# codelibs/ranklib

Measured on AMD Instinct MI355X. Metric: boosting rounds/sec (LambdaMART -ranker 6, NDCG@10), higher is better.
Workload: dtype int64 fixed-point histograms + f64 lambdas/scores (f32 leaf chains as in the Java)

## Files before the change

ranklib_amd/csrc/rl_internal.h:

```cpp
#pragma once
#include <hip/hip_runtime.h>
#include <stdint.h>

#include <string>
#include <vector>

#include "../../include/rlhip.h"

namespace rl {

constexpr int kThreads = 256;
constexpr int kWave = 64;
constexpr int kFinThreads = 320;
constexpr int kLog2Chunk = 14;
constexpr int kChunk = 1 << kLog2Chunk;
#ifndef RL_NODE_CHUNK
#define RL_NODE_CHUNK 8192
#endif
constexpr int kNodeChunk = RL_NODE_CHUNK;
constexpr int kMinChunk = 512;
#ifndef RL_HIST_DOCS
#define RL_HIST_DOCS 2
#endif
constexpr int kHistDocs = RL_HIST_DOCS;
#ifndef RL_LOOKBACK2
#define RL_LOOKBACK2 1
#endif
#ifndef RL_HIST_PREFETCH
#define RL_HIST_PREFETCH 0
#endif
constexpr int kHistFG = 16;
#ifndef RL_PART_TILE
#define RL_PART_TILE 2048
#endif
constexpr int kPartTile = RL_PART_TILE;
constexpr int kMaxBins = 4096;
constexpr int kHistLdsStride = 264;
constexpr int kHistLdsBytes = 64 * 1024;
#ifndef RL_KSPEC
#define RL_KSPEC 4
#endif
constexpr int kSpec = RL_KSPEC;
constexpr int kLambdaWaveCap = 384;
constexpr int kLambdaBlockCap = 5000;
#ifndef RL_RANK_SHORT
#define RL_RANK_SHORT 384
#endif
constexpr int kRankShort = RL_RANK_SHORT;
constexpr int kLambdaFusedMaxK = 16;

struct NodeRec {
    int32_t start, count;
    int32_t buf, parent;
    int32_t left, right;
    int32_t best_f, best_t;
    double  best_S;
    double  deviance;
    double  sum_response;
    double  sq_response;
    long long tot_hi; unsigned long long tot_lo;
    long long sq;
    float   output; int32_t gcount;
    int32_t pl, pr;
    int32_t fid;
    int32_t prepared;
    int32_t best_cl, tie;
    unsigned long long ph;
    long long best_hi; unsigned long long best_lo;
};

struct SlotRec {
// ... 166 lines not shown
```

ranklib_amd/csrc/rl_k_rank.inc:

```

namespace rl {

template <int G>
__device__ __forceinline__ void group_sync()
{
    if (G > kWave) __syncthreads();
    else { __builtin_amdgcn_fence(__ATOMIC_ACQ_REL, "workgroup"); __builtin_amdgcn_wave_barrier(); }
}

constexpr int kRankLdsPerDoc = 20;
struct RankArgs {
    const double *scores; const float *labels; const int *qoff; const double *ideal; const double *disc;
    double *ss; float *sl; int *srel; int *sidx;
    double *ndcg; int k;
    int metric;
    int *aux_i; double *aux_a, *aux_b;
    double err_max;
    const int *rd_ext;
};

__device__ __forceinline__ double err_R(int rel, double mx) { return (double)java_pow2m1(rel) / mx; }

__device__ __forceinline__ bool metric_binary_view(int metric) { return metric == RL_METRIC_MAP || metric == RL_METRIC_P || metric == RL_METRIC_RR; }
__device__ void rank_metric(const RankArgs &a, int qi, int cur, int n, int size, const int *s_rel)
{
    const bool is_map = a.metric == RL_METRIC_MAP;
    {
        double res = 0.0;
        if (a.metric == RL_METRIC_NDCG) {
            const double ideal = a.ideal[qi];
            if (n > 0 && ideal > 0.0) {
                double dcg = 0;
                for (int i = 0; i < size; i++) dcg += gain_of(s_rel[i]) * a.disc[i];
// ... 18 lines not shown
            int first = -1, second = -1;
            for (int i = 0; i < rsize && second < 0; i++)
                if (s_rel[i]) { if (first < 0) first = i; else second = i; }
            res = (first < 0) ? 0.0 : (double)(1.0f / (float)(first + 1));
            if (a.aux_i) { a.aux_i[2 * qi] = first; a.aux_i[2 * qi + 1] = second; }
        } else {
            double sc = 0.0, p = 1.0;
            for (int i = 1; i <= size; i++) { const double R = err_R(s_rel[i - 1], a.err_max); sc += p * R / i; p *= (1.0 - R); }
            res = sc;
            if (a.aux_a) {
                const int ssize = (n > a.k) ? a.k : n;
                double pp = 1.0;
                for (int i = 0; i < ssize; i++) {
                    const double R = err_R(s_rel[i], a.err_max), np = pp * (1.0 - R);
                    pp *= np;
                    a.aux_a[cur + i] = R; a.aux_b[cur + i] = np;
                }
            }
        }
        a.ndcg[qi] = res;
    }
}

template <int G, int CAP>
__device__ void rank_query(const RankArgs &a, int qi, int tid, double *s_raw, int *s_rel, float *s_lab, int *s_idx)
{
    int cur = a.qoff[qi], n = a.qoff[qi + 1] - cur;
    if (G >= kWave) {
        cur = __builtin_amdgcn_readfirstlane(cur); n = __builtin_amdgcn_readfirstlane(n);
    }
    for (int i = tid; i < n; i += G) s_raw[i] = a.scores[cur + i];
    group_sync<G>();
    int size = a.k;
    if (a.k > n || a.k <= 0) size = n;
    const bool is_map = a.metric == RL_METRIC_MAP, bin_view = metric_binary_view(a.metric);
    constexpr int PER = (CAP + G - 1) / G;
    double v[PER]; float l[PER]; int pos[PER];
#pragma unroll
    for (int u = 0; u < PER; u++) {
        const int r = tid + u * G;
        pos[u] = 0; v[u] = 0.0; l[u] = 0.f;
        if (G >= kWave) {
            const int rb = __builtin_amdgcn_readfirstlane(r);
            if (rb >= n) break;
            v[u] = (r < n) ? s_raw[r] : 0.0;
            const int j0 = rb, j1 = min(rb + 64, n);
            int p = 0;
#pragma unroll 8
            for (int j = 0; j < j0; j++) p += (s_raw[j] >= v[u]) ? 1 : 0;
#pragma unroll 8
            for (int j = j0; j < j1; j++) { const double x = s_raw[j]; p += ((x > v[u]) || (x == v[u] && j < r)) ? 1 : 0; }
#pragma unroll 8
            for (int j = j1; j < n; j++) p += (s_raw[j] > v[u]) ? 1 : 0;
            pos[u] = p;
            if (r < n) l[u] = a.labels[cur + r];
        } else if (r < n) {
            v[u] = s_raw[r];
            int p = 0;
            for (int j = 0; j < n; j++) { const double x = s_raw[j]; p += (x > v[u]) || (x == v[u] && j < r); }
            pos[u] = p; l[u] = a.labels[cur + r];
        }
    }
    group_sync<G>();
#pragma unroll
    for (int u = 0; u < PER; u++) {
        const int r = tid + u * G;
        if (r < n) {
            s_raw[pos[u]] = v[u]; s_rel[pos[u]] = bin_view ? (l[u] > 0.f ? 1 : 0) : (int)l[u];
            if (a.ss) { s_lab[pos[u]] = l[u]; s_idx[pos[u]] = r; }
        }
    }
    group_sync<G>();
    if (a.ss)
        for (int i = tid; i < n; i += G) { const float lv = s_lab[i]; a.ss[cur + i] = s_raw[i]; a.sl[cur + i] = lv; a.srel[cur + i] = (int)lv; a.sidx[cur + i] = s_idx[i]; }
    group_sync<G>();
    if (is_map) {
        if (tid == 0) { int count = 0; for (int i = 0; i < n; i++) { const int r = s_rel[i]; count += r; s_rel[i] = (count << 1) | r; } }
        group_sync<G>();
        for (int i = tid; i < n; i += G) {
            const int e = s_rel[i], cnt = e >> 1;
            if (a.aux_i) a.aux_i[cur + i] = cnt;
            s_raw[i] = (e & 1) ? ((double)cnt) / (i + 1) : 0.0;
        }
        group_sync<G>();
        if (tid == 0) {
            double ap = 0.0;
            for (int i = 0; i < n; i++) ap += s_raw[i];
            const int count = (n > 0) ? (s_rel[n - 1] >> 1) : 0;
            const int rdc = a.rd_ext ? a.rd_ext[qi] : count;
            a.ndcg[qi] = (rdc == 0) ? 0.0 : ap / rdc;
        }
        return;
    }
    if (G >= kWave && size <= kWave && (a.metric == RL_METRIC_NDCG || a.metric == RL_METRIC_DCG)) {
        if (tid < kWave) {
            const double term = (tid < size) ? gain_of(s_rel[tid]) * a.disc[tid] : 0.0;
            const double ideal = (a.metric == RL_METRIC_NDCG) ? a.ideal[qi] : 1.0;
            double dcg = 0;
            for (int i = 0; i < size; i++) dcg += readlane_f64(term, i);
            double res = dcg;
            if (a.metric == RL_METRIC_NDCG) res = (n > 0 && ideal > 0.0) ? dcg / ideal : 0.0;
            if (tid == 0) a.ndcg[qi] = res;
        }
        return;
    }
    if (tid == 0) rank_metric(a, qi, cur, n, size, s_rel);
}

__global__ __launch_bounds__(kThreads) void k_rank_wave(const RankArgs a, const int *qlist, int nq, int cap)
{
    constexpr int CAP = kLambdaWaveCap;
    extern __shared__ unsigned char smem_raw[];
    const int wave = threadIdx.x >> 6;
    const int slot = blockIdx.x * 4 + wave;
    if (slot >= nq) return;
    const int qi = qlist ? qlist[slot] : slot;
    unsigned char *base = smem_raw + (size_t)wave * ((size_t)cap * kRankLdsPerDoc);
    rank_query<kWave, CAP>(a, qi, lane_id(), (double *)base, (int *)(base + (size_t)cap * 8), (float *)(base + (size_t)cap * 12), (int *)(base + (size_t)cap * 16));
}

constexpr int kRankTinyDocs = 16, kRankTinyGroups = 16;
__global__ __launch_bounds__(kRankTinyDocs * kRankTinyGroups) void k_rank_tiny(const RankArgs a, const int *qlist, int nq)
{
    __shared__ unsigned char sm[kRankTinyGroups * kRankTinyDocs * kRankLdsPerDoc];
    const int grp = threadIdx.x / kRankTinyDocs;
    const int slot = blockIdx.x * kRankTinyGroups + grp;
    if (slot >= nq) return;
    unsigned char *base = sm + (size_t)grp * (kRankTinyDocs * kRankLdsPerDoc);
    rank_query<kRankTinyDocs, kRankTinyDocs>(a, qlist[slot], threadIdx.x % kRankTinyDocs, (double *)base, (int *)(base + kRankTinyDocs * 8), (float *)(base + kRankTinyDocs * 12),
                                             (int *)(base + kRankTinyDocs * 16));
}

constexpr int kRankBlockThreads = 1024;
constexpr int kRankHugeTile = 4096, kRankHugeDocs = 8;
__global__ __launch_bounds__(kRankBlockThreads) void k_rank_huge(const RankArgs a, const int *qlist, int nq, int *rel_scratch)
{
    __shared__ double tile[kRankHugeTile];
    if ((int)blockIdx.x >= nq) return;
    const int qi = qlist[blockIdx.x], tid = threadIdx.x;
    const int cur = a.qoff[qi], n = a.qoff[qi + 1] - cur;
    int size = a.k;
    if (a.k > n || a.k <= 0) size = n;
    const bool bin_view = metric_binary_view(a.metric);
    int *s_rel = rel_scratch + cur;
    for (int base = 0; base < n; base += kRankBlockThreads * kRankHugeDocs) {
        double v[kRankHugeDocs]; int r[kRankHugeDocs], pos[kRankHugeDocs];
#pragma unroll
        for (int u = 0; u < kRankHugeDocs; u++) { r[u] = base + tid + u * kRankBlockThreads; v[u] = r[u] < n ? a.scores[cur + r[u]] : 0.0; pos[u] = 0; }
        for (int t0 = 0; t0 < n; t0 += kRankHugeTile) {
            __syncthreads();
            const int m = min(kRankHugeTile, n - t0);
            for (int j = tid; j < m; j += kRankBlockThreads) tile[j] = a.scores[cur + t0 + j];
            __syncthreads();
            for (int j = 0; j < m; j++) {
                const double x = tile[j];
#pragma unroll
                for (int u = 0; u < kRankHugeDocs; u++) pos[u] += (x > v[u]) || (x == v[u] && t0 + j < r[u]);
            }
        }
#pragma unroll
        for (int u = 0; u < kRankHugeDocs; u++) {
            if (r[u] >= n) continue;
            const float l = a.labels[cur + r[u]];
            s_rel[pos[u]] = bin_view ? (l > 0.f ? 1 : 0) : (int)l;
            if (a.ss) { a.ss[cur + pos[u]] = v[u]; a.sl[cur + pos[u]] = l; a.srel[cur + pos[u]] = (int)l; a.sidx[cur + pos[u]] = r[u]; }
        }
    }
    __syncthreads();
    if (tid == 0) rank_metric(a, qi, cur, n, size, s_rel);
}

__global__ __launch_bounds__(kRankBlockThreads) void k_rank_block(const RankArgs a, const int *qlist, int nq, int cap)
{
    constexpr int CAP = kLambdaBlockCap;
    extern __shared__ unsigned char smem_raw[];
    if ((int)blockIdx.x >= nq) return;
    rank_query<kRankBlockThreads, CAP>(a, qlist[blockIdx.x], threadIdx.x, (double *)smem_raw, (int *)(smem_raw + (size_t)cap * 8), (float *)(smem_raw + (size_t)cap * 12),
                                       (int *)(smem_raw + (size_t)cap * 16));
}

__global__ __launch_bounds__(kRankBlockThreads) void k_rank_mixed(const RankArgs a, const int *qbig, int nbig, int cap_big, const int *qsmall, int nsmall, int cap)
{
    extern __shared__ unsigned char smem_raw[];
    if ((int)blockIdx.x < nbig) {
        rank_query<kRankBlockThreads, kLambdaBlockCap>(a, qbig[blockIdx.x], threadIdx.x, (double *)smem_raw, (int *)(smem_raw + (size_t)cap_big * 8),
                                                       (float *)(smem_raw + (size_t)cap_big * 12), (int *)(smem_raw + (size_t)cap_big * 16));
        return;
    }
    const int wave = threadIdx.x >> 6;
    const int slot = ((int)blockIdx.x - nbig) * (kRankBlockThreads / 64) + wave;
    if (slot >= nsmall) return;
    unsigned char *base = smem_raw + (size_t)wave * ((size_t)cap * kRankLdsPerDoc);
    rank_query<kWave, kLambdaWaveCap>(a, qsmall[slot], lane_id(), (double *)base, (int *)(base + (size_t)cap * 8), (float *)(base + (size_t)cap * 12), (int *)(base + (size_t)cap * 16));
}

}
```

ranklib_amd/csrc/rl_launch.inc:

```

namespace rl {

static int launch_rank(rl_trainer *t, DataSet &d, const double *scores, double *out, bool ranked)
{
    RankArgs a{scores, d.d_labels, d.d_qoff, d.d_ideal1, t->ctx.disc,
               ranked ? d.d_ss : nullptr, ranked ? d.d_sl : nullptr, ranked ? d.d_srel : nullptr, ranked ? d.d_sidx : nullptr,
               out, t->p.metric_k, t->p.metric, ranked ? d.d_aux_i : nullptr, ranked ? d.d_aux_a : nullptr, ranked ? d.d_aux_b : nullptr, t->err_max,
               d.d_ext_rd};
    if (d.n_tiny > 0) {
        t->arms[RL_ARM_RANK_TINY]++;
        hipLaunchKernelGGL(k_rank_tiny, dim3((d.n_tiny + kRankTinyGroups - 1) / kRankTinyGroups), dim3(kRankTinyDocs * kRankTinyGroups), 0, t->stream, a,
                           (const int *)d.d_qtiny, d.n_tiny);
    }
    if (!t->knobs.rank_split && d.n_big > 0 && d.n_small > 0) {
        const int wpb = kRankBlockThreads / 64;
        const size_t lds = std::max((size_t)d.max_big, (size_t)wpb * kLambdaWaveCap) * kRankLdsPerDoc;
        t->arms[RL_ARM_RANK_MIXED]++; t->arms[RL_ARM_RANK_HUGE] += d.n_huge > 0 ? 1 : 0;
        hipLaunchKernelGGL(k_rank_mixed, dim3(d.n_big + (d.n_small + wpb - 1) / wpb), dim3(kRankBlockThreads), lds, t->stream, a, (const int *)d.d_qbig, d.n_big, d.max_big,
                           (const int *)d.d_qsmall, d.n_small, kLambdaWaveCap);
        if (d.n_huge > 0)
            hipLaunchKernelGGL(k_rank_huge, dim3(d.n_huge), dim3(kRankBlockThreads), 0, t->stream, a, (const int *)d.d_qhuge, d.n_huge, d.d_relscratch);
        RL_HIP(hipGetLastError());
        return RL_OK;
    }
    t->arms[RL_ARM_RANK_WAVE_LONG] += d.n_small_long > 0 ? 1 : 0; t->arms[RL_ARM_RANK_WAVE_SHORT] += d.n_small > d.n_small_long ? 1 : 0;
    t->arms[RL_ARM_RANK_BLOCK] += d.n_big > 0 ? 1 : 0; t->arms[RL_ARM_RANK_HUGE] += d.n_huge > 0 ? 1 : 0;
    if (d.n_small_long > 0)
        hipLaunchKernelGGL(k_rank_wave, dim3((d.n_small_long + 3) / 4), dim3(kThreads), 4 * kLambdaWaveCap * kRankLdsPerDoc, t->stream, a,
                           (const int *)d.d_qsmall, d.n_small_long, kLambdaWaveCap);
    if (d.n_small > d.n_small_long)
        hipLaunchKernelGGL(k_rank_wave, dim3((d.n_small - d.n_small_long + 3) / 4), dim3(kThreads), 4 * kRankShort * kRankLdsPerDoc, t->stream, a,
                           (const int *)d.d_qsmall + d.n_small_long, d.n_small - d.n_small_long, kRankShort);
    if (d.n_big > 0)
        hipLaunchKernelGGL(k_rank_block, dim3(d.n_big), dim3(kRankBlockThreads), (size_t)d.max_big * kRankLdsPerDoc, t->stream, a, d.d_qbig, d.n_big, d.max_big);
    if (d.n_huge > 0)
        hipLaunchKernelGGL(k_rank_huge, dim3(d.n_huge), dim3(kRankBlockThreads), 0, t->stream, a, (const int *)d.d_qhuge, d.n_huge, d.d_relscratch);
    RL_HIP(hipGetLastError());
    return RL_OK;
}

template <bool ROOT>
static void launch_hist(const Ctx &c, const Knobs &kn, int64_t *arms, int gx, int gy, size_t lds, hipStream_t s, bool fq = false)
// ... 59 lines not shown
```

ranklib_amd/csrc/rl_round.inc:

```

namespace rl {

struct RoundPlan {
    size_t hist_lds, red_lds, par_lds, fin_lds, slot_words;
    int hist_gx, rootCs, rootChunks, nodes_in_lds, jbg, steps;
};

static int round_plan(const rl_trainer *t, RoundPlan &pl)
{
    const Ctx &c = t->ctx;
    pl.hist_lds = (size_t)c.sub * ((c.sub == 16 && c.TS <= kHistLdsStride) ? kHistLdsStride : c.TS) * 12;
    pl.hist_gx = c.numFG * (kHistFG / c.sub);
    pl.red_lds = (size_t)c.TS * 20;
    pl.rootCs = std::min(kChunk, std::max(kMinChunk, (((c.N + 63) / 64 + 255) & ~255)));
    pl.rootChunks = (c.N + pl.rootCs - 1) / pl.rootCs;
    pl.nodes_in_lds = (select_lds_bytes(c.L, c.NC, true, c.F, c.fs_on != 0) <= 60 * 1024) ? 1 : 0;
    pl.par_lds = (c.TS <= kParCacheTS) ? (size_t)c.TS * 20 + 8 : 0;
    pl.fin_lds = std::max((size_t)c.TS * (c.java ? 28 : 20) + 8 + pl.par_lds, select_lds_bytes(c.L, c.NC, pl.nodes_in_lds != 0, c.F, c.fs_on != 0));
    pl.jbg = (c.TS + 63) / 64;
    if (pl.fin_lds > 128 * 1024) return fail(RL_ERR_UNSUPPORTED, "too many features / leaves for the growth bookkeeping in LDS (feature sampling needs 64 bytes per feature)");
    pl.steps = std::max(c.L - 1, 1);
    pl.slot_words = (size_t)c.F * c.TS * c.limb_words + 4;
    return RL_OK;
}
// ... 287 lines not shown
        return RL_OK;
    }
    if (t->p.flags & RL_FLAG_FAST_LEAF) {
        const FastLeafArgs fa{c.lw, c.idx[0], c.idx[1], t->d_seg_buf, c.leaf_start, &c.st->n_leaves, c.MAXN + 1, stream_scores ? c.leaf_of : nullptr,
                              t->d_fast_part, (int32_t)t->fast_slots, t->d_fast_sums, c.nodes, c.leaf_node, c.mart};
        hipLaunchKernelGGL(k_fast_leaf_tiles, dim3((unsigned)t->fast_slots), dim3(kFastTile), 0, s, fa);
        hipLaunchKernelGGL(k_fast_leaf_finish, dim3((unsigned)(c.MAXN + 1)), dim3(kFastTile), 0, s, fa);
        return RL_OK;
    }
    const ChainSource src{nullptr, nullptr, c.lw, c.idx[0], c.idx[1], t->d_seg_buf, stream_scores ? c.leaf_of : nullptr};
    const ChainBufs *sums = &t->leaf_chain;
    if (t->dist && t->piece_chains) {
        int rcp = enqueue_leaf_chains_pieces(t, src);
        if (rcp) return rcp;
    } else if (t->dist) {
        int rco = enqueue_leaf_chains_owner(t, src);
        if (rco) return rco;
        sums = &t->gchain;
    } else enqueue_chain(t, t->leaf_chain, src);
    hipLaunchKernelGGL(k_leaf_output, dim3((c.L + kThreads - 1) / kThreads), dim3(kThreads), 0, s, c, *sums);
    return RL_OK;
}

static int enqueue_scores_and_metrics(rl_trainer *t, bool stream_scores, bool export_tree = true)
{
    Ctx &c = t->ctx;
    hipStream_t s = t->stream;
    const int m = t->round;
    if (stream_scores) hipLaunchKernelGGL(k_score_stream, dim3(std::max(1, std::min(2048, (c.N + kScoreBatch * kThreads - 1) / (kScoreBatch * kThreads)))), dim3(kThreads), 0, s, c);
    else hipLaunchKernelGGL(k_score_update, dim3(std::max(1, std::min(4096, (c.N + kScoreBatch * kThreads - 1) / (kScoreBatch * kThreads)))), dim3(kThreads), 0, s, c);
    if (export_tree) hipLaunchKernelGGL(k_export_tree, dim3(1), dim3(kThreads), 0, s, c, t->ens, m);
    RL_HIP(hipGetLastError());
    const bool use_side = !t->has_valid;
    if (use_side && t->side_pending) RL_HIP(hipStreamWaitEvent(s, t->ev_metric, 0));
    int rc = launch_rank(t, t->tr, c.scores, t->tr.d_ndcg, true);
    if (rc != RL_OK) return rc;
    if (use_side) {
        const double *mq = t->tr.d_ndcg; int mQ = t->tr.Q;
        if (t->dist) { rc = gather_queries(t, t->tr.d_ndcg, &mq); if (rc != RL_OK) return rc; mQ = t->Qglobal; }
        RL_HIP(hipEventRecord(t->ev_ranked, s));
        RL_HIP(hipStreamWaitEvent(t->side, t->ev_ranked, 0));
        enqueue_metric_mean(t, mq, mQ, c.round_metric + 2 * (size_t)m, t->side);
        RL_HIP(hipEventRecord(t->ev_metric, t->side));
        t->side_pending = true;
    } else if (t->dist) {
        const double *gq = nullptr;
        rc = gather_queries(t, t->tr.d_ndcg, &gq);
        if (rc != RL_OK) return rc;
        enqueue_metric_mean(t, gq, t->Qglobal, c.round_metric + 2 * (size_t)m);
    } else enqueue_metric_mean(t, t->tr.d_ndcg, t->tr.Q, c.round_metric + 2 * (size_t)m);
    if (t->has_valid) {
        hipLaunchKernelGGL(k_valid_update, dim3(std::min<int64_t>(4096, (t->va.N + kThreads - 1) / kThreads)), dim3(kThreads), 0, s,
                           t->ens, c.MAXN, m, (const float *)t->va.d_X, (int)t->va.N, t->F, c.lr, t->va.d_scores);
        rc = launch_rank(t, t->va, t->va.d_scores, t->va.d_ndcg, false);
        if (rc != RL_OK) return rc;
        if (t->dist) {
            const double *gq = nullptr;
            rc = gather_queries(t, t->va.d_ndcg, &gq, true);
            if (rc != RL_OK) return rc;
            enqueue_metric_mean(t, gq, t->vQglobal, c.round_metric + 2 * (size_t)m + 1);
        } else enqueue_metric_mean(t, t->va.d_ndcg, t->va.Q, c.round_metric + 2 * (size_t)m + 1);
    }
    RL_HIP(hipGetLastError());
    t->round = m + 1;
    t->n_kept = t->round;
    return RL_OK;
// ... 1 lines not shown

static bool round_streams_scores(const rl_trainer *t)
{
    const Ctx &c = t->ctx;
    return t->knobs.score_stream && !(t->p.flags & RL_FLAG_SERIAL_CHAIN) && c.leaf_of != nullptr && c.L > 0 && c.L <= 1024;
}

static int enqueue_round(rl_trainer *t)
{
    Ctx &c = t->ctx;
    const int tie_mode = c.tie_on;
    struct TieModeRestore { Ctx &c; int v; ~TieModeRestore() { c.tie_on = v; } } tie_mode_restore{c, tie_mode};
    const bool stream_scores = round_streams_scores(t);
    RoundPlan pl;
    int rc = round_plan(t, pl);
    if (rc) return rc;
    int n_max = 0;
    bool root_quant_fused = false;
    if ((rc = enqueue_lambdas(t, n_max)) != RL_OK) return rc;
    if ((rc = enqueue_max_and_quant(t, n_max, root_quant_fused)) != RL_OK) return rc;
    for (;;) {
        if ((rc = enqueue_root(t, pl, root_quant_fused)) != RL_OK) return rc;
        root_quant_fused = false;
        Growth g(c);
        if ((rc = grow_tree(t, pl, g)) != RL_OK) return rc;
        if ((rc = enqueue_leaf_outputs(t, stream_scores)) != RL_OK) return rc;
        if (!c.tie_on || !g.defer_seen) break;
        bool other_cut = false;
        if ((rc = resolve_ties(t, pl.fin_lds, pl.nodes_in_lds, true, &other_cut)) != RL_OK) return rc;
        if (!other_cut || !(c.tie_on & 2)) break;
        c.tie_on = 1; t->tie_regrown++;
    }
    return enqueue_scores_and_metrics(t, stream_scores);
}

}
```

ranklib_amd/csrc/rl_trainer.hip:

```cpp
#include <algorithm>
#include <chrono>
#include <cmath>
#include <limits>
#include <cstdio>
#include <cstring>
#include <map>
#include <memory>

#include "rl_internal.h"
#include "rl_lists_host.h"
#include "rl_knobs.h"
#include "rl_device.h"
#include "rl_wave.h"
#include "rl_kernels_init.inc"
#include "rl_chain.inc"
#include "rl_kernels_round.inc"
#include "rl_fast_leaf.inc"
#include "rl_step2.inc"
#include "rl_java_order.inc"
#include "rl_csc.inc"
#include "rl_tie.inc"
#include "rl_membench.inc"
#include "rl_dist.inc"
#include "rl_model.h"

namespace rl {

static thread_local std::string g_err;
static double g_err_max = 16.0;
void set_error(const std::string &msg) { g_err = msg; }
int fail(int code, const std::string &msg) { g_err = msg; return code; }

struct DataSet : ListSetHost {
    float *d_X = nullptr;
    int64_t rows_next = -1;
    float *d_labels = nullptr; int32_t *d_qoff = nullptr; double *d_ideal0 = nullptr, *d_ideal1 = nullptr;
    double *d_scores = nullptr, *d_ndcg = nullptr;
    double *d_ss = nullptr; float *d_sl = nullptr; int32_t *d_srel = nullptr, *d_sidx = nullptr, *d_docq = nullptr;
    int32_t *d_aux_i = nullptr; double *d_aux_a = nullptr, *d_aux_b = nullptr;
    int32_t *d_ext_rd = nullptr;
    int32_t *d_qsmall = nullptr, *d_qbig = nullptr, *d_qtiny = nullptr; int32_t n_small = 0, n_big = 0, n_tiny = 0, max_big = 0, n_small_long = 0; bool all_small = false;
    int32_t *d_qhuge = nullptr, *d_relscratch = nullptr; int32_t n_huge = 0;
    int32_t *d_qcls[5] = {nullptr, nullptr, nullptr, nullptr, nullptr}; int32_t n_qcls[5] = {0, 0, 0, 0, 0};
};

struct TimingSlot { double ms = 0; int64_t launches = 0; double bytes = 0; };

}

using namespace rl;

struct rl_trainer {
    rl_params p;
    Knobs knobs;
    int32_t F = 0;
    std::vector<int32_t> feature_ids;
    std::vector<int32_t> vcol;
    DataSet tr, va;
    bool has_train = false, has_valid = false, inited = false, finished = false;
    hipStream_t stream = nullptr;
    hipStream_t side = nullptr; hipEvent_t ev_ranked = nullptr, ev_metric = nullptr; bool side_pending = false;
    hipStream_t lam_s[3] = {nullptr, nullptr, nullptr}; hipEvent_t ev_lam_fork = nullptr, ev_lam_join[3] = {nullptr, nullptr, nullptr};
    DevPool pool;
    Ctx ctx;
    EnsTree ens;
    int32_t L_eff = 0;
    int32_t *d_tie_flag = nullptr;
    int64_t sp_entries = 0; int32_t sp_cols = 0;
    int32_t cr_groups = 0; double cr_entries = 0, cr_overflow = 0;
    double err_max = 16.0;
    int32_t round = 0;
    int64_t refit_stats[3] = {0, 0, 0};
    int64_t arms[RL_ARM_COUNT_] = {};
    unsigned long long *h_progress = nullptr; uint32_t tree_seq = 0;
    unsigned long long chain_seq = 0; std::vector<void *> pinned;
    int32_t synced_rounds = 0;
    long long tie_stalls = 0, tie_nodes = 0, tie_chain_nodes = 0, tie_chain_docs = 0;
    long long tie_batches = 0;
    bool fin_split = false;
    long long tie_phase_us[6] = {0, 0, 0, 0, 0, 0};
    long long chain_calls[2] = {0, 0}, chain_repairs[2] = {0, 0}, chain_timeouts = 0, chain_wait_us = 0;
    long long tie_regrown = 0;
    long long tie_us = 0, tie_spec_segs = 0, tie_spec_miss = 0, tie_spec_serial = 0, tie_spec_repairs = 0;
    std::vector<int32_t> h_nthr; std::vector<char> tie_blob;
// ... 75 lines not shown
    }
    d.n_huge = (int32_t)huge.size();
    if (!huge.empty()) {
        RL_HIP(t->pool.alloc(&d.d_qhuge, huge.size()));
        RL_HIP(hipMemcpy(d.d_qhuge, huge.data(), huge.size() * sizeof(int32_t), hipMemcpyHostToDevice));
        RL_HIP(t->pool.alloc(&d.d_relscratch, (size_t)d.N));
    }
    if (tiny.size() < tiny_min) { small.insert(small.end(), tiny.begin(), tiny.end()); tiny.clear(); }
    d.n_tiny = (int32_t)tiny.size();
    RL_HIP(t->pool.alloc(&d.d_qtiny, tiny.size()));
    if (!tiny.empty()) RL_HIP(hipMemcpy(d.d_qtiny, tiny.data(), tiny.size() * sizeof(int32_t), hipMemcpyHostToDevice));
    auto by_len = [&](int32_t a, int32_t b) { return (d.qoff[a + 1] - d.qoff[a]) > (d.qoff[b + 1] - d.qoff[b]); };
    std::stable_sort(small.begin(), small.end(), by_len);
    std::stable_sort(big.begin(), big.end(), by_len);
    d.n_small = (int32_t)small.size(); d.n_big = (int32_t)big.size();
    d.n_small_long = 0;
    for (int32_t q : small) d.n_small_long += (d.qoff[q + 1] - d.qoff[q] > kRankShort) ? 1 : 0;
    d.max_big = big.empty() ? 0 : (((d.qoff[big[0] + 1] - d.qoff[big[0]]) + 63) & ~63);
    d.all_small = false;
    RL_HIP(t->pool.alloc(&d.d_qsmall, small.size()));
    RL_HIP(t->pool.alloc(&d.d_qbig, big.size()));
    if (!small.empty()) RL_HIP(hipMemcpy(d.d_qsmall, small.data(), small.size() * sizeof(int32_t), hipMemcpyHostToDevice));
    if (!big.empty()) RL_HIP(hipMemcpy(d.d_qbig, big.data(), big.size() * sizeof(int32_t), hipMemcpyHostToDevice));
    std::vector<int32_t> qcls[5];
    for (int32_t q = 0; q < d.Q; q++) {
        const int n = d.qoff[q + 1] - d.qoff[q];
        qcls[n <= kLambdaTinyDocs ? 4 : n <= 64 ? 0 : n <= 128 ? 1 : n <= 192 ? 2 : 3].push_back(q);
    }
    if (qcls[4].size() < tiny_min) {
        qcls[0].insert(qcls[0].end(), qcls[4].begin(), qcls[4].end());
        qcls[4].clear();
    }
    for (int cI = 0; cI < 5; cI++) {
        std::stable_sort(qcls[cI].begin(), qcls[cI].end(), by_len);
        d.n_qcls[cI] = (int32_t)qcls[cI].size();
        RL_HIP(t->pool.alloc(&d.d_qcls[cI], qcls[cI].size()));
        if (!qcls[cI].empty()) RL_HIP(hipMemcpy(d.d_qcls[cI], qcls[cI].data(), qcls[cI].size() * sizeof(int32_t), hipMemcpyHostToDevice));
    }
    return RL_OK;
}

static int next_pow2(int v) { int p = 1; while (p < v) p <<= 1; return p; }

static hipEvent_t take_event(rl_trainer *t)
{
    if (!t->ev_free.empty()) { hipEvent_t e = t->ev_free.back(); t->ev_free.pop_back(); return e; }
// ... 34 lines not shown

static int gather_queries(rl_trainer *t, const double *local, const double **out, bool valid = false)
{
    hipStream_t s = t->stream;
    const int Q = valid ? t->va.Q : t->tr.Q, Qmax = valid ? t->vQmax : t->Qmax;
    double *snd = valid ? t->d_vqsend : t->d_qsend, *gat = valid ? t->d_vqgath : t->d_qgath, *cat = valid ? t->d_vqcat : t->d_qcat;
    hipLaunchKernelGGL(k_copy_f64, dim3(std::max(1, std::min(1024, (Q + kThreads - 1) / kThreads))), dim3(kThreads), 0, s, local, snd, Q);
    int rc = t->dist->allgather(snd, gat, (size_t)Qmax * sizeof(double), s);
    if (rc) return rc;
    hipLaunchKernelGGL(k_concat_ranks, dim3(64), dim3(kThreads), 0, s, (const double *)gat, (const int32_t *)(valid ? t->d_vallQ : t->d_allQ), t->n_ranks, Qmax, cat);
    *out = cat;
    return RL_OK;
}

}

#include "rl_tie_host.inc"
#include "rl_round.inc"

namespace rl {

static int sync_rounds(rl_trainer *t)
{
    RL_HIP(hipStreamSynchronize(t->stream));
    RL_HIP(hipStreamSynchronize(t->side));
    collect_timing(t);
    TreeState st;
    RL_HIP(hipMemcpy(&st, t->ctx.st, sizeof(st), hipMemcpyDeviceToHost));
    if (st.error) return fail(RL_ERR_HIP, "device tree growth ran out of node slots (internal error)");
    if (t->round > t->synced_rounds) {
        t->h_metrics.resize((size_t)t->round * 2);
        RL_HIP(hipMemcpy(t->h_metrics.data() + 2 * (size_t)t->synced_rounds, t->ctx.round_metric + 2 * (size_t)t->synced_rounds,
                         (size_t)(t->round - t->synced_rounds) * 2 * sizeof(float), hipMemcpyDeviceToHost));
        t->synced_rounds = t->round;
    }
    return RL_OK;
}

static int fetch_tree(const rl_trainer *tc, int i, HostTree &out)
{
    rl_trainer *t = const_cast<rl_trainer *>(tc);
    if ((int)t->trees.size() <= i) t->trees.resize((size_t)i + 1);
    if (t->trees[i].n_nodes > 0) { out = t->trees[i]; return RL_OK; }
    const int MAXN = t->ctx.MAXN;
    int32_t nn = 0;
    RL_HIP(hipMemcpy(&nn, t->ens.n_nodes + i, sizeof(int32_t), hipMemcpyDeviceToHost));
// ... 128 lines not shown
    RL_HIP(hipFuncSetAttribute((const void *)k_hist<true, 16, kHistLdsStride, true, true>, hipFuncAttributeMaxDynamicSharedMemorySize, kHistLdsBytes));
    RL_HIP(hipFuncSetAttribute((const void *)k_hist<false, 16, kHistLdsStride, true, true>, hipFuncAttributeMaxDynamicSharedMemorySize, kHistLdsBytes));
    RL_HIP(hipFuncSetAttribute((const void *)k_hist<true, 16, 0>, hipFuncAttributeMaxDynamicSharedMemorySize, kHistLdsBytes));
    RL_HIP(hipFuncSetAttribute((const void *)k_hist<false, 16, 0>, hipFuncAttributeMaxDynamicSharedMemorySize, kHistLdsBytes));
    RL_HIP(hipFuncSetAttribute((const void *)k_hist<true, 8, 0>, hipFuncAttributeMaxDynamicSharedMemorySize, kHistLdsBytes));
    RL_HIP(hipFuncSetAttribute((const void *)k_hist<false, 8, 0>, hipFuncAttributeMaxDynamicSharedMemorySize, kHistLdsBytes));
    RL_HIP(hipFuncSetAttribute((const void *)k_hist<true, 4, 0>, hipFuncAttributeMaxDynamicSharedMemorySize, kHistLdsBytes));
    RL_HIP(hipFuncSetAttribute((const void *)k_hist<false, 4, 0>, hipFuncAttributeMaxDynamicSharedMemorySize, kHistLdsBytes));
    RL_HIP(hipFuncSetAttribute((const void *)k_hist<true, 2, 0>, hipFuncAttributeMaxDynamicSharedMemorySize, kHistLdsBytes));
    RL_HIP(hipFuncSetAttribute((const void *)k_hist<false, 2, 0>, hipFuncAttributeMaxDynamicSharedMemorySize, kHistLdsBytes));
    RL_HIP(hipFuncSetAttribute((const void *)k_hist<true, 1, 0>, hipFuncAttributeMaxDynamicSharedMemorySize, kHistLdsBytes));
    RL_HIP(hipFuncSetAttribute((const void *)k_hist<false, 1, 0>, hipFuncAttributeMaxDynamicSharedMemorySize, kHistLdsBytes));
    RL_HIP(hipFuncSetAttribute((const void *)k_hist_reduce, hipFuncAttributeMaxDynamicSharedMemorySize, kMaxBins * 20));
    RL_HIP(hipFuncSetAttribute((const void *)k_hist_sp<kHistLdsStride>, hipFuncAttributeMaxDynamicSharedMemorySize, kHistFG * kHistLdsStride * 8));
    RL_HIP(hipFuncSetAttribute((const void *)k_select, hipFuncAttributeMaxDynamicSharedMemorySize, 128 * 1024));
    RL_HIP(hipFuncSetAttribute((const void *)k_hist_finish_wide, hipFuncAttributeMaxDynamicSharedMemorySize, 128 * 1024));
    RL_HIP(hipFuncSetAttribute((const void *)k_hist_finish<true, false>, hipFuncAttributeMaxDynamicSharedMemorySize, 128 * 1024));
    RL_HIP(hipFuncSetAttribute((const void *)k_hist_finish<false, false>, hipFuncAttributeMaxDynamicSharedMemorySize, 128 * 1024));
    RL_HIP(hipFuncSetAttribute((const void *)k_hist_finish<true, true>, hipFuncAttributeMaxDynamicSharedMemorySize, 128 * 1024));
    RL_HIP(hipFuncSetAttribute((const void *)k_hist_finish<false, true>, hipFuncAttributeMaxDynamicSharedMemorySize, 128 * 1024));
    RL_HIP(hipFuncSetAttribute((const void *)k_hist_finish<true, false, true>, hipFuncAttributeMaxDynamicSharedMemorySize, 128 * 1024));
    RL_HIP(hipFuncSetAttribute((const void *)k_hist_finish<false, false, true>, hipFuncAttributeMaxDynamicSharedMemorySize, 128 * 1024));
    RL_HIP(hipFuncSetAttribute((const void *)k_rank_block, hipFuncAttributeMaxDynamicSharedMemorySize, ((kLambdaBlockCap + 63) & ~63) * kRankLdsPerDoc));
    RL_HIP(hipFuncSetAttribute((const void *)k_rank_mixed, hipFuncAttributeMaxDynamicSharedMemorySize, std::max((kLambdaBlockCap + 63) & ~63, (kRankBlockThreads / 64) * kLambdaWaveCap) * kRankLdsPerDoc));
    RL_HIP(hipFuncSetAttribute((const void *)k_lambda_tiny, hipFuncAttributeMaxDynamicSharedMemorySize, kLambdaTinyGroups * lambda_tiny_group_bytes(kLambdaFusedMaxK)));
    RL_HIP(hipFuncSetAttribute((const void *)k_lambda_fused<256, 0>, hipFuncAttributeMaxDynamicSharedMemorySize, kLambdaFusedMaxK * (256 + 8) * 16 + 2048));
    RL_HIP(hipFuncSetAttribute((const void *)k_lambda_fused<256, 0, true>, hipFuncAttributeMaxDynamicSharedMemorySize, kLambdaFusedMaxK * (256 + 8) * 16 + 2048 + lambda_fused_cp_bytes(kLambdaFusedMaxK, 256)));
    RL_HIP(hipFuncSetAttribute((const void *)k_lambda_fused<256, 1>, hipFuncAttributeMaxDynamicSharedMemorySize, kLambdaFusedMaxK * (256 + 8) * 16 + 8192));
    RL_HIP(hipFuncSetAttribute((const void *)k_lambda_fused<256, 2>, hipFuncAttributeMaxDynamicSharedMemorySize, kLambdaFusedMaxK * (256 + 8) * 16 + 8192));
    RL_HIP(hipFuncSetAttribute((const void *)k_lambda_fused<256, 3>, hipFuncAttributeMaxDynamicSharedMemorySize, kLambdaFusedMaxK * (256 + 8) * 16 + 2048));
    RL_HIP(hipFuncSetAttribute((const void *)k_lambda_fused<256, 4>, hipFuncAttributeMaxDynamicSharedMemorySize, kLambdaFusedMaxK * (256 + 8) * 16 + 2048));
    RL_HIP(hipFuncSetAttribute((const void *)k_chain_stitch, hipFuncAttributeMaxDynamicSharedMemorySize, 160 * 1024));
    RL_HIP(hipFuncSetAttribute((const void *)k_tie_finish, hipFuncAttributeMaxDynamicSharedMemorySize, 128 * 1024));
    *out = t.release();
    return RL_OK;
}

void rl_destroy(rl_trainer *t)
{
    if (!t) return;
    (void)hipSetDevice(t->p.device);
    if (t->knobs.tie_prof && t->tie_stalls > 0)
        fprintf(stderr, "[rlhip] tie-break: %lld resolutions (%lld batches, %lld trees regrown), host us: first read %lld, chains %lld, candidates+lists %lld, sums %lld, finish %lld, total %lld\n",
                t->tie_stalls, t->tie_batches, t->tie_regrown, t->tie_phase_us[0], t->tie_phase_us[1], t->tie_phase_us[2], t->tie_phase_us[3], t->tie_phase_us[4], t->tie_us);
    if (t->knobs.chain_prof)
        fprintf(stderr, "[rlhip] float chains: %lld watched evaluations with %lld repair passes, %lld blind ones with %lld; progress-word time-outs %lld; host waited %lld us for stitches\n",
                t->chain_calls[0], t->chain_repairs[0], t->chain_calls[1], t->chain_repairs[1], t->chain_timeouts, t->chain_wait_us);
// ... 527 lines not shown
```

Measured before the change: 367.1.

## Pack short queries into rank blocks, shrink rank LDS, vectorize rank counting, defer metric mean

Short queries for the mixed rank kernel are now packed host-side into blocks by actual length, using precomputed slot descriptors instead of a fixed per-wave capacity. Per-doc LDS drops from 20 to 16 bytes by reusing the index array for relevance, which lets two blocks share a CU. The rank-position counting loop reads scores as double2 pairs with unrolled per-unit spans, padding odd-length queries with -inf. Enqueueing the metric mean on the side stream is deferred to the next round or sync so it overlaps later work. Together these should raise rank-kernel occupancy and cut per-round overhead, but they add packing logic and alignment and padding assumptions.

```diff
diff --git a/ranklib_amd/csrc/rl_internal.h b/ranklib_amd/csrc/rl_internal.h
--- a/ranklib_amd/csrc/rl_internal.h
+++ b/ranklib_amd/csrc/rl_internal.h
@@ -6,6 +6,7 @@
 #include <vector>
 
 #include "../../include/rlhip.h"
+#include "rl_rank_pack_host.h"
 
 namespace rl {
 
@@ -47,6 +48,7 @@
 #define RL_RANK_SHORT 384
 #endif
 constexpr int kRankShort = RL_RANK_SHORT;
+static_assert(kRankPackDocs >= ((kLambdaBlockCap + 63) & ~63) && 2 * kRankPackDocs * kRankLdsPerDoc <= 160 * 1024, "two blocks of k_rank_mixed share a CU's LDS");
 constexpr int kLambdaFusedMaxK = 16;
 
 struct NodeRec {
diff --git a/ranklib_amd/csrc/rl_k_rank.inc b/ranklib_amd/csrc/rl_k_rank.inc
--- a/ranklib_amd/csrc/rl_k_rank.inc
+++ b/ranklib_amd/csrc/rl_k_rank.inc
@@ -8,7 +8,6 @@
     else { __builtin_amdgcn_fence(__ATOMIC_ACQ_REL, "workgroup"); __builtin_amdgcn_wave_barrier(); }
 }
 
-constexpr int kRankLdsPerDoc = 20;
 struct RankArgs {
     const double *scores; const float *labels; const int *qoff; const double *ideal; const double *disc;
     double *ss; float *sl; int *srel; int *sidx;
@@ -73,14 +72,51 @@
     }
 }
 
+template <int PER, int NU>
+__device__ __forceinline__ void count_span(const double *s_raw, int j0, int j1, int lo, int hi, int r, const double (&v)[PER], int (&p)[PER])
+{
+#pragma unroll 4
+    for (int j = j0; j < j1; j += 2) {
+        const double2 x = *(const double2 *)(s_raw + j);
+#pragma unroll
+        for (int u = 0; u < NU; u++) {
+            if (u < lo) { p[u] += (x.x > v[u]) ? 1 : 0; p[u] += (x.y > v[u]) ? 1 : 0; }
+            else if (u >= hi) { p[u] += (x.x >= v[u]) ? 1 : 0; p[u] += (x.y >= v[u]) ? 1 : 0; }
+            else {
+                p[u] += ((x.x > v[u]) || (x.x == v[u] && j < r)) ? 1 : 0;
+                p[u] += ((x.y > v[u]) || (x.y == v[u] && j + 1 < r)) ? 1 : 0;
+            }
+        }
+    }
+}
+
+template <int G, int PER, int NU>
+__device__ __forceinline__ void rank_count(const double *s_raw, int n, int rb0, int r0, const double (&v)[PER], int (&p)[PER])
+{
+#pragma unroll
+    for (int s = 0; s < NU; s++) {
+        const int w0 = rb0 + s * G;
+        if (G > kWave) count_span<PER, NU>(s_raw, s == 0 ? 0 : w0 - G + kWave, w0, s, s, 0, v, p);
+        count_span<PER, NU>(s_raw, w0, min(w0 + kWave, n), s, s + 1, r0 + s * G, v, p);
+    }
+    if (G > kWave) count_span<PER, NU>(s_raw, rb0 + (NU - 1) * G + kWave, n, NU, NU, 0, v, p);
+}
+
+template <int G, int PER, int NU = 1>
+__device__ __forceinline__ void rank_count_nu(int nu, const double *s_raw, int n, int rb0, int r0, const double (&v)[PER], int (&p)[PER])
+{
+    if (nu == NU) rank_count<G, PER, NU>(s_raw, n, rb0, r0, v, p);
+    else if constexpr (NU < PER) rank_count_nu<G, PER, NU + 1>(nu, s_raw, n, rb0, r0, v, p);
+}
+
 template <int G, int CAP>
-__device__ void rank_query(const RankArgs &a, int qi, int tid, double *s_raw, int *s_rel, float *s_lab, int *s_idx)
-{
-    int cur = a.qoff[qi], n = a.qoff[qi + 1] - cur;
+__device__ void rank_query(const RankArgs &a, int qi, int cur, int n, int tid, double *s_raw, float *s_lab, int *s_idx)
+{
     if (G >= kWave) {
         cur = __builtin_amdgcn_readfirstlane(cur); n = __builtin_amdgcn_readfirstlane(n);
     }
     for (int i = tid; i < n; i += G) s_raw[i] = a.scores[cur + i];
+    if (G >= kWave && tid == 0 && (n & 1)) s_raw[n] = -__builtin_inf();
     group_sync<G>();
     int size = a.k;
     if (a.k > n || a.k <= 0) size = n;
@@ -88,28 +124,26 @@
     constexpr int PER = (CAP + G - 1) / G;
     double v[PER]; float l[PER]; int pos[PER];
 #pragma unroll
-    for (int u = 0; u < PER; u++) {
-        const int r = tid + u * G;
-        pos[u] = 0; v[u] = 0.0; l[u] = 0.f;
-        if (G >= kWave) {
-            const int rb = __builtin_amdgcn_readfirstlane(r);
-            if (rb >= n) break;
-            v[u] = (r < n) ? s_raw[r] : 0.0;
-            const int j0 = rb, j1 = min(rb + 64, n);
-            int p = 0;
-#pragma unroll 8
-            for (int j = 0; j < j0; j++) p += (s_raw[j] >= v[u]) ? 1 : 0;
-#pragma unroll 8
-            for (int j = j0; j < j1; j++) { const double x = s_raw[j]; p += ((x > v[u]) || (x == v[u] && j < r)) ? 1 : 0; }
-#pragma unroll 8
-            for (int j = j1; j < n; j++) p += (s_raw[j] > v[u]) ? 1 : 0;
-            pos[u] = p;
-            if (r < n) l[u] = a.labels[cur + r];
-        } else if (r < n) {
-            v[u] = s_raw[r];
-            int p = 0;
-            for (int j = 0; j < n; j++) { const double x = s_raw[j]; p += (x > v[u]) || (x == v[u] && j < r); }
-            pos[u] = p; l[u] = a.labels[cur + r];
+    for (int u = 0; u < PER; u++) { pos[u] = 0; v[u] = 0.0; l[u] = 0.f; }
+    if (G >= kWave) {
+        const int rb0 = __builtin_amdgcn_readfirstlane(tid);
+        const int nu = rb0 < n ? min((n - rb0 + G - 1) / G, PER) : 0;
+#pragma unroll
+        for (int u = 0; u < PER; u++) {
+            const int r = tid + u * G;
+            if (r < n) { v[u] = s_raw[r]; l[u] = a.labels[cur + r]; }
+        }
+        rank_count_nu<G, PER>(nu, s_raw, n, rb0, tid, v, pos);
+    } else {
+#pragma unroll
+        for (int u = 0; u < PER; u++) {
+            const int r = tid + u * G;
+            if (r < n) {
+                v[u] = s_raw[r];
+                int p = 0;
+                for (int j = 0; j < n; j++) { const double x = s_raw[j]; p += (x > v[u]) || (x == v[u] && j < r); }
+                pos[u] = p; l[u] = a.labels[cur + r];
+            }
         }
     }
     group_sync<G>();
@@ -117,13 +151,19 @@
     for (int u = 0; u < PER; u++) {
         const int r = tid + u * G;
         if (r < n) {
-            s_raw[pos[u]] = v[u]; s_rel[pos[u]] = bin_view ? (l[u] > 0.f ? 1 : 0) : (int)l[u];
+            s_raw[pos[u]] = v[u];
             if (a.ss) { s_lab[pos[u]] = l[u]; s_idx[pos[u]] = r; }
-        }
-    }
-    group_sync<G>();
+            else s_idx[pos[u]] = bin_view ? (l[u] > 0.f ? 1 : 0) : (int)l[u];
+        }
+    }
+    group_sync<G>();
+    int *s_rel = s_idx;
     if (a.ss)
-        for (int i = tid; i < n; i += G) { const float lv = s_lab[i]; a.ss[cur + i] = s_raw[i]; a.sl[cur + i] = lv; a.srel[cur + i] = (int)lv; a.sidx[cur + i] = s_idx[i]; }
+        for (int i = tid; i < n; i += G) {
+            const float lv = s_lab[i];
+            a.ss[cur + i] = s_raw[i]; a.sl[cur + i] = lv; a.srel[cur + i] = (int)lv; a.sidx[cur + i] = s_idx[i];
+            s_rel[i] = bin_view ? (lv > 0.f ? 1 : 0) : (int)lv;
+        }
     group_sync<G>();
     if (is_map) {
         if (tid == 0) { int count = 0; for (int i = 0; i < n; i++) { const int r = s_rel[i]; count += r; s_rel[i] = (count << 1) | r; } }
@@ -158,28 +198,34 @@
     if (tid == 0) rank_metric(a, qi, cur, n, size, s_rel);
 }
 
+template <int G, int CAP>
+__device__ __forceinline__ void rank_carved(const RankArgs &a, int qi, int cur, int n, int tid, unsigned char *base, int cap)
+{
+    rank_query<G, CAP>(a, qi, cur, n, tid, (double *)base, (float *)(base + (size_t)cap * 8), (int *)(base + (size_t)cap * 12));
+}
+
 __global__ __launch_bounds__(kThreads) void k_rank_wave(const RankArgs a, const int *qlist, int nq, int cap)
 {
     constexpr int CAP = kLambdaWaveCap;
-    extern __shared__ unsigned char smem_raw[];
+    extern __shared__ __align__(16) unsigned char smem_raw[];
     const int wave = threadIdx.x >> 6;
     const int slot = blockIdx.x * 4 + wave;
     if (slot >= nq) return;
     const int qi = qlist ? qlist[slot] : slot;
-    unsigned char *base = smem_raw + (size_t)wave * ((size_t)cap * kRankLdsPerDoc);
-    rank_query<kWave, CAP>(a, qi, lane_id(), (double *)base, (int *)(base + (size_t)cap * 8), (float *)(base + (size_t)cap * 12), (int *)(base + (size_t)cap * 16));
+    const int cur = a.qoff[qi], n = a.qoff[qi + 1] - cur;
+    rank_carved<kWave, CAP>(a, qi, cur, n, lane_id(), smem_raw + (size_t)wave * ((size_t)cap * kRankLdsPerDoc), cap);
 }
 
 constexpr int kRankTinyDocs = 16, kRankTinyGroups = 16;
 __global__ __launch_bounds__(kRankTinyDocs * kRankTinyGroups) void k_rank_tiny(const RankArgs a, const int *qlist, int nq)
 {
-    __shared__ unsigned char sm[kRankTinyGroups * kRankTinyDocs * kRankLdsPerDoc];
+    __shared__ __align__(16) unsigned char sm[kRankTinyGroups * kRankTinyDocs * kRankLdsPerDoc];
     const int grp = threadIdx.x / kRankTinyDocs;
     const int slot = blockIdx.x * kRankTinyGroups + grp;
     if (slot >= nq) return;
-    unsigned char *base = sm + (size_t)grp * (kRankTinyDocs * kRankLdsPerDoc);
-    rank_query<kRankTinyDocs, kRankTinyDocs>(a, qlist[slot], threadIdx.x % kRankTinyDocs, (double *)base, (int *)(base + kRankTinyDocs * 8), (float *)(base + kRankTinyDocs * 12),
-                                             (int *)(base + kRankTinyDocs * 16));
+    const int qi = qlist[slot];
+    const int cur = a.qoff[qi], n = a.qoff[qi + 1] - cur;
+    rank_carved<kRankTinyDocs, kRankTinyDocs>(a, qi, cur, n, threadIdx.x % kRankTinyDocs, sm + (size_t)grp * (kRankTinyDocs * kRankLdsPerDoc), kRankTinyDocs);
 }
 
 constexpr int kRankBlockThreads = 1024;
@@ -224,25 +270,27 @@
 __global__ __launch_bounds__(kRankBlockThreads) void k_rank_block(const RankArgs a, const int *qlist, int nq, int cap)
 {
     constexpr int CAP = kLambdaBlockCap;
-    extern __shared__ unsigned char smem_raw[];
+    extern __shared__ __align__(16) unsigned char smem_raw[];
     if ((int)blockIdx.x >= nq) return;
-    rank_query<kRankBlockThreads, CAP>(a, qlist[blockIdx.x], threadIdx.x, (double *)smem_raw, (int *)(smem_raw + (size_t)cap * 8), (float *)(smem_raw + (size_t)cap * 12),
-                                       (int *)(smem_raw + (size_t)cap * 16));
-}
-
-__global__ __launch_bounds__(kRankBlockThreads) void k_rank_mixed(const RankArgs a, const int *qbig, int nbig, int cap_big, const int *qsmall, int nsmall, int cap)
-{
-    extern __shared__ unsigned char smem_raw[];
+    const int qi = qlist[blockIdx.x];
+    const int cur = a.qoff[qi], n = a.qoff[qi + 1] - cur;
+    rank_carved<kRankBlockThreads, CAP>(a, qi, cur, n, threadIdx.x, smem_raw, cap);
+}
+
+__global__ __launch_bounds__(kRankBlockThreads, 8) void k_rank_mixed(const RankArgs a, const int *qbig, int nbig, int cap_big, const RankSlot *slots)
+{
+    extern __shared__ __align__(16) unsigned char smem_raw[];
     if ((int)blockIdx.x < nbig) {
-        rank_query<kRankBlockThreads, kLambdaBlockCap>(a, qbig[blockIdx.x], threadIdx.x, (double *)smem_raw, (int *)(smem_raw + (size_t)cap_big * 8),
-                                                       (float *)(smem_raw + (size_t)cap_big * 12), (int *)(smem_raw + (size_t)cap_big * 16));
+        const int qi = qbig[blockIdx.x];
+        const int cur = a.qoff[qi], n = a.qoff[qi + 1] - cur;
+        rank_carved<kRankBlockThreads, kLambdaBlockCap>(a, qi, cur, n, threadIdx.x, smem_raw, cap_big);
         return;
     }
     const int wave = threadIdx.x >> 6;
-    const int slot = ((int)blockIdx.x - nbig) * (kRankBlockThreads / 64) + wave;
-    if (slot >= nsmall) return;
-    unsigned char *base = smem_raw + (size_t)wave * ((size_t)cap * kRankLdsPerDoc);
-    rank_query<kWave, kLambdaWaveCap>(a, qsmall[slot], lane_id(), (double *)base, (int *)(base + (size_t)cap * 8), (float *)(base + (size_t)cap * 12), (int *)(base + (size_t)cap * 16));
-}
-
-}
+    const int4 s = ((const int4 *)slots)[((int)blockIdx.x - nbig) * kRankPackLists + wave];
+    if (s.x < 0) return;
+    const int n = __builtin_amdgcn_readfirstlane(s.z), off = __builtin_amdgcn_readfirstlane(s.w);
+    rank_carved<kWave, kLambdaWaveCap>(a, s.x, s.y, n, lane_id(), smem_raw + (size_t)off * kRankLdsPerDoc, rank_carve_docs(n));
+}
+
+}
diff --git a/ranklib_amd/csrc/rl_launch.inc b/ranklib_amd/csrc/rl_launch.inc
--- a/ranklib_amd/csrc/rl_launch.inc
+++ b/ranklib_amd/csrc/rl_launch.inc
@@ -13,11 +13,10 @@
                            (const int *)d.d_qtiny, d.n_tiny);
     }
     if (!t->knobs.rank_split && d.n_big > 0 && d.n_small > 0) {
-        const int wpb = kRankBlockThreads / 64;
-        const size_t lds = std::max((size_t)d.max_big, (size_t)wpb * kLambdaWaveCap) * kRankLdsPerDoc;
+        const size_t lds = (size_t)std::max(d.max_big, d.rank_block_docs) * kRankLdsPerDoc;
         t->arms[RL_ARM_RANK_MIXED]++; t->arms[RL_ARM_RANK_HUGE] += d.n_huge > 0 ? 1 : 0;
-        hipLaunchKernelGGL(k_rank_mixed, dim3(d.n_big + (d.n_small + wpb - 1) / wpb), dim3(kRankBlockThreads), lds, t->stream, a, (const int *)d.d_qbig, d.n_big, d.max_big,
-                           (const int *)d.d_qsmall, d.n_small, kLambdaWaveCap);
+        hipLaunchKernelGGL(k_rank_mixed, dim3(d.n_big + d.n_rank_blocks), dim3(kRankBlockThreads), lds, t->stream, a, (const int *)d.d_qbig, d.n_big, d.max_big,
+                           (const RankSlot *)d.d_rank_slots);
         if (d.n_huge > 0)
             hipLaunchKernelGGL(k_rank_huge, dim3(d.n_huge), dim3(kRankBlockThreads), 0, t->stream, a, (const int *)d.d_qhuge, d.n_huge, d.d_relscratch);
         RL_HIP(hipGetLastError());
diff --git a/ranklib_amd/csrc/rl_rank_pack_host.h b/ranklib_amd/csrc/rl_rank_pack_host.h
--- /dev/null
+++ b/ranklib_amd/csrc/rl_rank_pack_host.h
@@ -0,0 +1,48 @@
+#pragma once
+#include <algorithm>
+#include <cstdint>
+#include <vector>
+
+namespace rl {
+
+constexpr int kRankLdsPerDoc = 16;
+constexpr int kRankPackLists = 16;
+constexpr int kRankPackDocs = 5056;
+constexpr int rank_carve_docs(int n) { return (n + 3) & ~3; }
+
+struct RankPack {
+    std::vector<int32_t> first, count;
+    std::vector<int32_t> off;
+    int32_t max_docs = 0;
+};
+
+inline RankPack rank_pack(const std::vector<int32_t> &len, int budget_docs)
+{
+    RankPack pk;
+    pk.off.resize(len.size());
+    int32_t used = 0, held = 0;
+    for (size_t i = 0; i < len.size(); i++) {
+        const int32_t need = rank_carve_docs(len[i]);
+        if (held == kRankPackLists || (held > 0 && used + need > budget_docs)) { used = 0; held = 0; }
+        if (held == 0) { pk.first.push_back((int32_t)i); pk.count.push_back(0); }
+        pk.off[i] = used;
+        used += need; held++;
+        pk.count.back() = held;
+        pk.max_docs = std::max(pk.max_docs, used);
+    }
+    return pk;
+}
+
+struct RankSlot { int32_t q, cur, n, off; };
+inline std::vector<RankSlot> rank_slots(const RankPack &pk, const std::vector<int32_t> &lists, const std::vector<int32_t> &qoff)
+{
+    std::vector<RankSlot> s(pk.first.size() * kRankPackLists, RankSlot{-1, 0, 0, 0});
+    for (size_t b = 0; b < pk.first.size(); b++)
+        for (int32_t w = 0; w < pk.count[b]; w++) {
+            const int32_t i = pk.first[b] + w, q = lists[i];
+            s[b * kRankPackLists + w] = RankSlot{q, qoff[q], qoff[q + 1] - qoff[q], pk.off[i]};
+        }
+    return s;
+}
+
+}
diff --git a/ranklib_amd/csrc/rl_round.inc b/ranklib_amd/csrc/rl_round.inc
--- a/ranklib_amd/csrc/rl_round.inc
+++ b/ranklib_amd/csrc/rl_round.inc
@@ -333,11 +333,23 @@
     return RL_OK;
 }
 
+static int flush_metric_mean(rl_trainer *t)
+{
+    if (!t->metric_due_out) return RL_OK;
+    RL_HIP(hipStreamWaitEvent(t->side, t->ev_ranked, 0));
+    enqueue_metric_mean(t, t->metric_due_q, t->metric_due_n, t->metric_due_out, t->side);
+    RL_HIP(hipEventRecord(t->ev_metric, t->side));
+    t->metric_due_out = nullptr;
+    return RL_OK;
+}
+
 static int enqueue_scores_and_metrics(rl_trainer *t, bool stream_scores, bool export_tree = true)
 {
     Ctx &c = t->ctx;
     hipStream_t s = t->stream;
     const int m = t->round;
+    int rcf = flush_metric_mean(t);
+    if (rcf != RL_OK) return rcf;
     if (stream_scores) hipLaunchKernelGGL(k_score_stream, dim3(std::max(1, std::min(2048, (c.N + kScoreBatch * kThreads - 1) / (kScoreBatch * kThreads)))), dim3(kThreads), 0, s, c);
     else hipLaunchKernelGGL(k_score_update, dim3(std::max(1, std::min(4096, (c.N + kScoreBatch * kThreads - 1) / (kScoreBatch * kThreads)))), dim3(kThreads), 0, s, c);
     if (export_tree) hipLaunchKernelGGL(k_export_tree, dim3(1), dim3(kThreads), 0, s, c, t->ens, m);
@@ -350,9 +362,7 @@
         const double *mq = t->tr.d_ndcg; int mQ = t->tr.Q;
         if (t->dist) { rc = gather_queries(t, t->tr.d_ndcg, &mq); if (rc != RL_OK) return rc; mQ = t->Qglobal; }
         RL_HIP(hipEventRecord(t->ev_ranked, s));
-        RL_HIP(hipStreamWaitEvent(t->side, t->ev_ranked, 0));
-        enqueue_metric_mean(t, mq, mQ, c.round_metric + 2 * (size_t)m, t->side);
-        RL_HIP(hipEventRecord(t->ev_metric, t->side));
+        t->metric_due_q = mq; t->metric_due_n = mQ; t->metric_due_out = c.round_metric + 2 * (size_t)m;
         t->side_pending = true;
     } else if (t->dist) {
         const double *gq = nullptr;
@@ -400,6 +410,7 @@
     for (;;) {
         if ((rc = enqueue_root(t, pl, root_quant_fused)) != RL_OK) return rc;
         root_quant_fused = false;
+        if ((rc = flush_metric_mean(t)) != RL_OK) return rc;
         Growth g(c);
         if ((rc = grow_tree(t, pl, g)) != RL_OK) return rc;
         if ((rc = enqueue_leaf_outputs(t, stream_scores)) != RL_OK) return rc;
diff --git a/ranklib_amd/csrc/rl_trainer.hip b/ranklib_amd/csrc/rl_trainer.hip
--- a/ranklib_amd/csrc/rl_trainer.hip
+++ b/ranklib_amd/csrc/rl_trainer.hip
@@ -40,6 +40,7 @@
     int32_t *d_aux_i = nullptr; double *d_aux_a = nullptr, *d_aux_b = nullptr;
     int32_t *d_ext_rd = nullptr;
     int32_t *d_qsmall = nullptr, *d_qbig = nullptr, *d_qtiny = nullptr; int32_t n_small = 0, n_big = 0, n_tiny = 0, max_big = 0, n_small_long = 0; bool all_small = false;
+    RankSlot *d_rank_slots = nullptr; int32_t n_rank_blocks = 0, rank_block_docs = 0;
     int32_t *d_qhuge = nullptr, *d_relscratch = nullptr; int32_t n_huge = 0;
     int32_t *d_qcls[5] = {nullptr, nullptr, nullptr, nullptr, nullptr}; int32_t n_qcls[5] = {0, 0, 0, 0, 0};
 };
@@ -60,6 +61,7 @@
     bool has_train = false, has_valid = false, inited = false, finished = false;
     hipStream_t stream = nullptr;
     hipStream_t side = nullptr; hipEvent_t ev_ranked = nullptr, ev_metric = nullptr; bool side_pending = false;
+    const double *metric_due_q = nullptr; int metric_due_n = 0; float *metric_due_out = nullptr;
     hipStream_t lam_s[3] = {nullptr, nullptr, nullptr}; hipEvent_t ev_lam_fork = nullptr, ev_lam_join[3] = {nullptr, nullptr, nullptr};
     DevPool pool;
     Ctx ctx;
@@ -181,6 +183,14 @@
     RL_HIP(t->pool.alloc(&d.d_qbig, big.size()));
     if (!small.empty()) RL_HIP(hipMemcpy(d.d_qsmall, small.data(), small.size() * sizeof(int32_t), hipMemcpyHostToDevice));
     if (!big.empty()) RL_HIP(hipMemcpy(d.d_qbig, big.data(), big.size() * sizeof(int32_t), hipMemcpyHostToDevice));
+    {
+        std::vector<int32_t> len(small.size());
+        for (size_t i = 0; i < small.size(); i++) len[i] = d.qoff[small[i] + 1] - d.qoff[small[i]];
+        const RankPack pk = rank_pack(len, kRankPackDocs);
+        const std::vector<RankSlot> slots = rank_slots(pk, small, d.qoff);
+        d.n_rank_blocks = (int32_t)pk.first.size(); d.rank_block_docs = pk.max_docs;
+        RL_HIP(t->pool.upload(&d.d_rank_slots, slots.data(), slots.size()));
+    }
     std::vector<int32_t> qcls[5];
     for (int32_t q = 0; q < d.Q; q++) {
         const int n = d.qoff[q + 1] - d.qoff[q];
@@ -261,6 +271,8 @@
 
 static int sync_rounds(rl_trainer *t)
 {
+    int rcf = flush_metric_mean(t);
+    if (rcf != RL_OK) return rcf;
     RL_HIP(hipStreamSynchronize(t->stream));
     RL_HIP(hipStreamSynchronize(t->side));
     collect_timing(t);
@@ -435,7 +447,7 @@
     RL_HIP(hipFuncSetAttribute((const void *)k_hist_finish<true, false, true>, hipFuncAttributeMaxDynamicSharedMemorySize, 128 * 1024));
     RL_HIP(hipFuncSetAttribute((const void *)k_hist_finish<false, false, true>, hipFuncAttributeMaxDynamicSharedMemorySize, 128 * 1024));
     RL_HIP(hipFuncSetAttribute((const void *)k_rank_block, hipFuncAttributeMaxDynamicSharedMemorySize, ((kLambdaBlockCap + 63) & ~63) * kRankLdsPerDoc));
-    RL_HIP(hipFuncSetAttribute((const void *)k_rank_mixed, hipFuncAttributeMaxDynamicSharedMemorySize, std::max((kLambdaBlockCap + 63) & ~63, (kRankBlockThreads / 64) * kLambdaWaveCap) * kRankLdsPerDoc));
+    RL_HIP(hipFuncSetAttribute((const void *)k_rank_mixed, hipFuncAttributeMaxDynamicSharedMemorySize, kRankPackDocs * kRankLdsPerDoc));
     RL_HIP(hipFuncSetAttribute((const void *)k_lambda_tiny, hipFuncAttributeMaxDynamicSharedMemorySize, kLambdaTinyGroups * lambda_tiny_group_bytes(kLambdaFusedMaxK)));
     RL_HIP(hipFuncSetAttribute((const void *)k_lambda_fused<256, 0>, hipFuncAttributeMaxDynamicSharedMemorySize, kLambdaFusedMaxK * (256 + 8) * 16 + 2048));
     RL_HIP(hipFuncSetAttribute((const void *)k_lambda_fused<256, 0, true>, hipFuncAttributeMaxDynamicSharedMemorySize, kLambdaFusedMaxK * (256 + 8) * 16 + 2048 + lambda_fused_cp_bytes(kLambdaFusedMaxK, 256)));
```

Result: faster. 376.4, median of 6 (+2.5%).
